# qwerfdsaplking/SATrans

Measured on AMD Instinct MI355X. Metric: training samples/sec (AliCCP-shaped, emb=32, 3L/4H, meta_mode=QK), higher is better.
Workload: dtype f32; 1 GPU; BASELINE configs[1]: AliCCP-shaped SATrans training step, 19 fields, 6,571,961 table rows (841 MB fp32), uniform ids, dropout on, dense-Adam+L2 semantics over all rows; batch_per_gpu=8192, global_batch=8192, embedding_dim=32, layers=3, heads=4, fields=19, parallelism=dp1

## Files before the change

### satrans_amd/csrc/embed_adam.hip

```cpp
#include <algorithm>
#include <cstdlib>
#include <cstring>

#include <rocprim/rocprim.hpp>

#include "common.h"

namespace satrans {

constexpr int kChunk = 16;
constexpr int kStreamBlock = 256;
constexpr int kStreamBlocks = 2048;

struct AdamK {
    float neg_step, w1, beta2, w2, eps, l2x2, l2;
    double rbc2;
    float rbc2f;
    int fast;
};

__host__ inline AdamK make_adamk(const satrans_adam_hparams& h) {
    AdamK k;
    k.neg_step = -h.lr_over_bc1;
    k.rbc2 = 1.0 / (double)h.bc2_sqrt;
// ... 268 lines not shown
__device__ __forceinline__ void touched_apply_body(int64_t bid, double* s_red, float4* __restrict__ P, float4* __restrict__ M,
                                                   float4* __restrict__ V, const int32_t* __restrict__ sorted_rows,
                                                   int64_t n, const float4* __restrict__ rowsum,
                                                   const int32_t* __restrict__ head_of, const AdamK& k,
                                                   double* __restrict__ reg_partials, float4* __restrict__ G,
                                                   int32_t* __restrict__ last, int t) {
    const int64_t j = (bid * 256 + threadIdx.x) / LPR;
    const int q = threadIdx.x % LPR;
    double reg = 0.0;
    if (j < n && head_of[j] == 1) {
        const int64_t at = (int64_t)sorted_rows[j] * LPR + q;
        if (G) {
            G[at] = rowsum[j * LPR + q];
        } else {
            float4 p = P[at], m = M[at], v = V[at];
            reg += adam4(p, m, v, rowsum[j * LPR + q], k);
            P[at] = p; M[at] = m; V[at] = v;
            if (last && q == 0) last[sorted_rows[j]] = t;
        }
    }
    const double total = block_sum(reg, s_red);
    if (threadIdx.x == 0) reg_partials[bid] = total;
}

template <int LPR>
__device__ __forceinline__ void touched_finish_body(int64_t bid, double* s_red, float4* __restrict__ P, float4* __restrict__ M,
                                                    float4* __restrict__ V, int64_t chunks,
                                                    const float4* __restrict__ done_sum,
                                                    const int32_t* __restrict__ done_row, const AdamK& k,
                                                    double* __restrict__ reg_partials, float4* __restrict__ G,
                                                    int32_t* __restrict__ last, int t) {
    const int64_t c = (bid * 256 + threadIdx.x) / LPR;
    const int q = threadIdx.x % LPR;
    double reg = 0.0;
    if (c < chunks) {
        const int32_t row = done_row[c];
        if (row >= 0) {
            const int64_t at = (int64_t)row * LPR + q;
            if (G) {
                G[at] = done_sum[c * LPR + q];
            } else {
                float4 p = P[at], m = M[at], v = V[at];
                reg += adam4(p, m, v, done_sum[c * LPR + q], k);
                P[at] = p; M[at] = m; V[at] = v;
                if (last && q == 0) last[row] = t;
            }
        }
    }
    const double total = block_sum(reg, s_red);
    if (threadIdx.x == 0) reg_partials[bid] = total;
}

template <int LPR>
__device__ __forceinline__ void touched_spans_body(int64_t bid, double* s_red, float4* __restrict__ P, float4* __restrict__ M,
                                                   float4* __restrict__ V, int64_t chunks,
                                                   const float4* __restrict__ partial,
                                                   const int32_t* __restrict__ info,
                                                   const int32_t* __restrict__ trail_row, const AdamK& k,
                                                   double* __restrict__ reg_partials, float4* __restrict__ G,
                                                   int32_t* __restrict__ last, int t) {
    const int64_t group = (bid * 256 + threadIdx.x) / LPR;
    const int q = threadIdx.x % LPR;
    double reg = 0.0;
    if (group < chunks && (info[group] & 1)) {
        float4 acc = partial[(group * 2 + 1) * LPR + q];
        for (int64_t c = group + 1; c < chunks; ++c) {
            const int f = info[c];
            if (!(f & 2)) break;
            const float4 g = partial[(c * 2 + 0) * LPR + q];
            acc.x += g.x; acc.y += g.y; acc.z += g.z; acc.w += g.w;
            if (f & 4) break;
        }
        const int64_t at = (int64_t)trail_row[group] * LPR + q;
        if (G) {
            G[at] = acc;
        } else {
            float4 p = P[at], m = M[at], v = V[at];
            reg += adam4(p, m, v, acc, k);
            P[at] = p; M[at] = m; V[at] = v;
            if (last && q == 0) last[trail_row[group]] = t;
        }
    }
    const double total = block_sum(reg, s_red);
    if (threadIdx.x == 0) reg_partials[bid] = total;
}

template <int LPR>
__global__ __launch_bounds__(256) void touched_step_kernel(int64_t sblocks, int64_t cblocks, float4* __restrict__ P,
                                                          float4* __restrict__ M, float4* __restrict__ V, AdamK k,
                                                          float4* __restrict__ G, int32_t* __restrict__ last, int t,
                                                          const int32_t* __restrict__ sorted_rows, int64_t n,
                                                          const float4* __restrict__ rowsum, const int32_t* __restrict__ head_of,
                                                          double* __restrict__ reg_apply, int64_t chunks,
                                                          const float4* __restrict__ done_sum, const int32_t* __restrict__ done_row,
                                                          double* __restrict__ reg_finish, int64_t supers,
                                                          const float4* __restrict__ partial2, const int32_t* __restrict__ info2,
                                                          const int32_t* __restrict__ trail_row2, double* __restrict__ reg_spans) {
    __builtin_amdgcn_s_setprio(3);
    __shared__ double s_red[256];
    const int64_t b = blockIdx.x;
    if (b < sblocks)
        touched_spans_body<LPR>(b, s_red, P, M, V, supers, partial2, info2, trail_row2, k, reg_spans, G, last, t);
    else if (b < sblocks + cblocks)
        touched_finish_body<LPR>(b - sblocks, s_red, P, M, V, chunks, done_sum, done_row, k, reg_finish, G, last, t);
    else
        touched_apply_body<LPR>(b - sblocks - cblocks, s_red, P, M, V, sorted_rows, n, rowsum, head_of, k, reg_apply, G, last, t);
}

template <int LPR>
__global__ __launch_bounds__(256) void adam_rows_kernel(float4* __restrict__ P, float4* __restrict__ M,
                                                       float4* __restrict__ V, int64_t row0, int64_t rows,
                                                       const float4* __restrict__ G, int32_t* __restrict__ last, int t,
                                                       AdamK k, double* __restrict__ reg_partials) {
    __shared__ double s_red[256];
    const int64_t i = (int64_t)blockIdx.x * 256 + threadIdx.x;
    double reg = 0.0;
    if (i < rows * LPR) {
        const int64_t at = row0 * LPR + i;
        float4 p = P[at], m = M[at], v = V[at];
        reg = adam4(p, m, v, G[i], k);
        P[at] = p; M[at] = m; V[at] = v;
        if (last && i % LPR == 0) last[row0 + i / LPR] = t;
    }
    const double total = block_sum(reg, s_red);
    if (threadIdx.x == 0) reg_partials[blockIdx.x] = total;
}

template <int LPR>
__global__ void pack_rows_kernel(const int32_t* __restrict__ src, int64_t n, const float4* __restrict__ gemb,
                                 float4* __restrict__ out) {
    const int64_t i = (int64_t)blockIdx.x * blockDim.x + threadIdx.x;
    if (i >= n * LPR) return;
    out[i] = gemb[(int64_t)src[i / LPR] * LPR + i % LPR];
}


struct LazyK {
    float w1, beta2, w2, eps, l2x2, l2;
    int fast;
};
__host__ inline LazyK make_lazyk(const satrans_adam_hparams& h) {
    LazyK k;
    k.fast = h.arith == SATRANS_ADAM_FAST ? 1 : 0;
    k.w1 = (float)(1.0 - (double)h.beta1);
    k.beta2 = h.beta2;
    k.w2 = (float)(1.0 - (double)h.beta2);
    k.eps = h.eps;
    k.l2 = h.l2;
    k.l2x2 = 2.0f * h.l2;
    return k;
}

using f32x2 = __attribute__((ext_vector_type(2))) float;

__device__ __forceinline__ f32x2 pk_fma(f32x2 a, f32x2 b, f32x2 c) { return __builtin_elementwise_fma(a, b, c); }
__device__ __forceinline__ f32x2 pk_mul(f32x2 a, f32x2 b) {
#pragma clang fp contract(off)
    return a * b;
}
__device__ __forceinline__ f32x2 pk_add(f32x2 a, f32x2 b) {
#pragma clang fp contract(off)
    return a + b;
}
__device__ __forceinline__ f32x2 pk_sub(f32x2 a, f32x2 b) {
#pragma clang fp contract(off)
    return a - b;
}
__device__ __forceinline__ f32x2 pk_set(float x) { return f32x2{x, x}; }

constexpr float kPkVLo = 0x1p-100f, kPkVHi = 0x1p64f;
constexpr float kPkALo = 0x1p-80f, kPkAHi = 0x1p40f;
constexpr float kPkEpsLo = 0x1p-30f;

__device__ __forceinline__ f32x2 pk_sqrt_rn(f32x2 x) {
    const f32x2 r = {__builtin_amdgcn_rsqf(x.x), __builtin_amdgcn_rsqf(x.y)};
    f32x2 s = pk_mul(x, r);
    f32x2 h = pk_mul(r, pk_set(0.5f));
    const f32x2 e = pk_fma(-h, s, pk_set(0.5f));
    h = pk_fma(h, e, h);
    s = pk_fma(s, e, s);
    const f32x2 d = pk_fma(-s, s, x);
    return pk_fma(d, h, s);
}

__device__ __forceinline__ f32x2 pk_div_rn(f32x2 a, f32x2 b) {
    f32x2 r = {__builtin_amdgcn_rcpf(b.x), __builtin_amdgcn_rcpf(b.y)};
    const f32x2 e = pk_fma(-b, r, pk_set(1.0f));
    r = pk_fma(e, r, r);
    f32x2 q = pk_mul(a, r);
    f32x2 d = pk_fma(-b, q, a);
    q = pk_fma(d, r, q);
    d = pk_fma(-b, q, a);
    return pk_fma(d, r, q);
}

__device__ __forceinline__ f32x2 pk_sqrt_ext(f32x2 v) {
    const bool sx = v.x < kPkVLo, sy = v.y < kPkVLo;
    const f32x2 up = {sx ? 0x1p64f : 1.0f, sy ? 0x1p64f : 1.0f};
    const f32x2 dn = {sx ? 0x1p-32f : 1.0f, sy ? 0x1p-32f : 1.0f};
    return pk_mul(pk_sqrt_rn(pk_mul(v, up)), dn);
}

__device__ __forceinline__ f32x2 pk_div_ext(f32x2 a, f32x2 den, bool& redo_x, bool& redo_y) {
    const bool sx = fabsf(a.x) < kPkALo, sy = fabsf(a.y) < kPkALo;
    const f32x2 up = {sx ? 0x1p69f : 1.0f, sy ? 0x1p69f : 1.0f};
    const f32x2 dn = {sx ? 0x1p-69f : 1.0f, sy ? 0x1p-69f : 1.0f};
    const f32x2 qs = pk_div_rn(pk_mul(a, up), den);
    f32x2 q = pk_mul(qs, dn);
    redo_x = sx && a.x != 0.f && !(fabsf(qs.x) >= 0x1p-57f);
    redo_y = sy && a.y != 0.f && !(fabsf(qs.y) >= 0x1p-57f);
    q.x = a.x == 0.f ? a.x : q.x;
    q.y = a.y == 0.f ? a.y : q.y;
    return q;
}

__device__ __forceinline__ float denom_of(float root, double rbc2, float eps) {
    return __fadd_rn((float)__dmul_rn((double)root, rbc2), eps);
}

__device__ __forceinline__ void adam_step4(f32x2 (&p)[2], f32x2 (&m)[2], f32x2 (&v)[2], f32x2 (&sq)[2], float neg_step,
                                           double rbc2, const LazyK& k) {
    f32x2 a[2];
#pragma unroll
    for (int u = 0; u < 2; ++u) {
        sq[u] = pk_fma(p[u], p[u], sq[u]);
        const f32x2 g = pk_add(pk_set(0.f), pk_mul(pk_set(k.l2x2), p[u]));
        m[u] = pk_fma(pk_set(k.w1), pk_sub(g, m[u]), m[u]);
        v[u] = pk_fma(pk_mul(pk_set(k.w2), g), g, pk_mul(v[u], pk_set(k.beta2)));
        a[u] = pk_mul(pk_set(neg_step), m[u]);
    }
    const float vmin = fminf(__builtin_fminf(__builtin_fminf(v[0].x, v[0].y), v[1].x), v[1].y);
    const float vmax = fmaxf(__builtin_fmaxf(__builtin_fmaxf(v[0].x, v[0].y), v[1].x), v[1].y);
    const float amin = fminf(__builtin_fminf(__builtin_fminf(fabsf(a[0].x), fabsf(a[0].y)), fabsf(a[1].x)), fabsf(a[1].y));
    const float amax = fmaxf(__builtin_fmaxf(__builtin_fmaxf(fabsf(a[0].x), fabsf(a[0].y)), fabsf(a[1].x)), fabsf(a[1].y));
    const bool packed = vmin >= kPkVLo && vmax <= kPkVHi && amin >= kPkALo && amax <= kPkAHi && k.eps >= kPkEpsLo;
    if (__all(packed)) {
#pragma unroll
        for (int u = 0; u < 2; ++u) {
            const f32x2 root = pk_sqrt_rn(v[u]);
            const f32x2 den = {denom_of(root.x, rbc2, k.eps), denom_of(root.y, rbc2, k.eps)};
            p[u] = pk_add(p[u], pk_div_rn(a[u], den));
        }
        return;
    }
    const bool v_sane = v[0].x >= 0.f && v[0].y >= 0.f && v[1].x >= 0.f && v[1].y >= 0.f;
    if (__all(k.eps > 0.f && v_sane && a[0].x == 0.f && a[0].y == 0.f && a[1].x == 0.f && a[1].y == 0.f)) {
        p[0] = pk_add(p[0], a[0]);
        p[1] = pk_add(p[1], a[1]);
        return;
    }
    const bool lane_small = amax < 0x1p-60f;
    auto lane_ok = [&](float a_) { return lane_small || a_ == 0.f || fabsf(a_) >= kPkALo; };
    const bool by_lane = v_sane && vmin >= kPkVLo && vmax <= kPkVHi && amax <= kPkAHi && k.eps >= kPkEpsLo && lane_ok(a[0].x) &&
                         lane_ok(a[0].y) && lane_ok(a[1].x) && lane_ok(a[1].y);
    if (__all(by_lane)) {
        const f32x2 up = pk_set(lane_small ? 0x1p69f : 1.0f), dn = pk_set(lane_small ? 0x1p-69f : 1.0f);
        f32x2 q[2], den[2];
#pragma unroll
        for (int u = 0; u < 2; ++u) {
            const f32x2 root = pk_sqrt_rn(v[u]);
            den[u] = f32x2{denom_of(root.x, rbc2, k.eps), denom_of(root.y, rbc2, k.eps)};
            q[u] = pk_mul(pk_div_rn(pk_mul(a[u], up), den[u]), dn);
        }
        if (lane_small && fmaxf(fmaxf(den[0].x, den[0].y), fmaxf(den[1].x, den[1].y)) > 0x1p-23f) {
#pragma unroll
            for (int u = 0; u < 2; ++u) q[u] = f32x2{__fdiv_rn(a[u].x, den[u].x), __fdiv_rn(a[u].y, den[u].y)};
        }
#pragma unroll
        for (int u = 0; u < 2; ++u) {
            q[u].x = a[u].x == 0.f ? a[u].x : q[u].x;
            q[u].y = a[u].y == 0.f ? a[u].y : q[u].y;
            p[u] = pk_add(p[u], q[u]);
        }
        return;
    }
    auto ext_ok = [&](float a_, float v_) { return (a_ == 0.f && v_ >= 0.f) || (fabsf(a_) <= kPkAHi && v_ > 0.f && v_ <= kPkVHi); };
    const bool extended = ext_ok(a[0].x, v[0].x) && ext_ok(a[0].y, v[0].y) && ext_ok(a[1].x, v[1].x) && ext_ok(a[1].y, v[1].y) &&
                          k.eps >= kPkEpsLo;
    if (__all(extended)) {
#pragma unroll
        for (int u = 0; u < 2; ++u) {
            const f32x2 root = pk_sqrt_ext(v[u]);
            const f32x2 den = {denom_of(root.x, rbc2, k.eps), denom_of(root.y, rbc2, k.eps)};
            bool redo_x, redo_y;
            f32x2 q = pk_div_ext(a[u], den, redo_x, redo_y);
            if (redo_x) q.x = __fdiv_rn(a[u].x, den.x);
            if (redo_y) q.y = __fdiv_rn(a[u].y, den.y);
            p[u] = pk_add(p[u], q);
        }
        return;
    }
#pragma unroll
    for (int u = 0; u < 2; ++u) {
        p[u].x = __fadd_rn(p[u].x, __fdiv_rn(a[u].x, denom_of(sqrtf(v[u].x), rbc2, k.eps)));
        p[u].y = __fadd_rn(p[u].y, __fdiv_rn(a[u].y, denom_of(sqrtf(v[u].y), rbc2, k.eps)));
    }
}

__device__ __forceinline__ void adam_step4_fast(f32x2 (&p)[2], f32x2 (&m)[2], f32x2 (&v)[2], f32x2 (&sq)[2], float neg_step,
                                                float rbc2f, const LazyK& k) {
#pragma unroll
    for (int u = 0; u < 2; ++u) {
        sq[u] = pk_fma(p[u], p[u], sq[u]);
        const f32x2 g = pk_add(pk_set(0.f), pk_mul(pk_set(k.l2x2), p[u]));
        m[u] = pk_fma(pk_set(k.w1), pk_sub(g, m[u]), m[u]);
        v[u] = pk_fma(pk_mul(pk_set(k.w2), g), g, pk_mul(v[u], pk_set(k.beta2)));
        const f32x2 a = pk_mul(pk_set(neg_step), m[u]);
        const f32x2 root = {__builtin_amdgcn_sqrtf(v[u].x), __builtin_amdgcn_sqrtf(v[u].y)};
        const f32x2 den = pk_fma(root, pk_set(rbc2f), pk_set(k.eps));
        const f32x2 r = {__builtin_amdgcn_rcpf(den.x), __builtin_amdgcn_rcpf(den.y)};
        p[u] = pk_fma(a, r, p[u]);
    }
}

__device__ __forceinline__ double replay_element4(float4& P4, float4& M4, float4& V4, int from, int to,
                                                  const double2* __restrict__ table, const LazyK& k) {
    f32x2 p[2] = {{P4.x, P4.y}, {P4.z, P4.w}}, m[2] = {{M4.x, M4.y}, {M4.z, M4.w}}, v[2] = {{V4.x, V4.y}, {V4.z, V4.w}};
    f32x2 sq[2] = {{0.f, 0.f}, {0.f, 0.f}};
    if (k.fast) {
        for (int s = from + 1; s <= to; ++s) {
            const double2 hp = table[s];
            adam_step4_fast(p, m, v, sq, -(float)hp.x, (float)hp.y, k);
        }
    } else {
        for (int s = from + 1; s <= to; ++s) {
            const double2 hp = table[s];
            adam_step4(p, m, v, sq, -(float)hp.x, hp.y, k);
        }
    }
    P4 = make_float4(p[0].x, p[0].y, p[1].x, p[1].y);
    M4 = make_float4(m[0].x, m[0].y, m[1].x, m[1].y);
    V4 = make_float4(v[0].x, v[0].y, v[1].x, v[1].y);
    return (double)k.l2 * (((double)sq[0].x + (double)sq[0].y) + ((double)sq[1].x + (double)sq[1].y));
}

template <int D>
__global__ __launch_bounds__(256) void lazy_replay_kernel(float4* __restrict__ P, float4* __restrict__ M, float4* __restrict__ V,
                                                         int32_t* __restrict__ last, const int32_t* __restrict__ sorted_rows,
                                                         int64_t n, int target, const double2* __restrict__ table, LazyK k,
                                                         double* __restrict__ reg_partials, int64_t slots) {
    constexpr int LR = D / 4;
    __shared__ double s_red[256];
    const int64_t j = ((int64_t)blockIdx.x * 256 + threadIdx.x) / LR;
    const int c = threadIdx.x % LR;
    double reg = 0.0;
    if (j < n) {
        const int32_t row = sorted_rows[j];
        const bool head = j == 0 || sorted_rows[j - 1] != row;
        if (head) {
            const int from = last[row];
            if (from < target) {
                const int64_t at = (int64_t)row * LR + c;
                float4 p = P[at], m = M[at], v = V[at];
                reg = replay_element4(p, m, v, from, target, table, k);
                P[at] = p; M[at] = m; V[at] = v;
            }
        }
    }
    __syncthreads();
    if (j < n && c == 0) {
        const int32_t row = sorted_rows[j];
        if ((j == 0 || sorted_rows[j - 1] != row) && last[row] < target) last[row] = target;
    }
    const double total = block_sum(reg, s_red);
    if (threadIdx.x == 0) {
        reg_partials[blockIdx.x] = total;
        for (int64_t t = (int64_t)blockIdx.x + gridDim.x; t < slots; t += gridDim.x) reg_partials[t] = 0.0;
    }
}

template <int D>
__global__ __launch_bounds__(256) void lazy_flush_kernel(float4* __restrict__ P, float4* __restrict__ M, float4* __restrict__ V,
                                                        int32_t* __restrict__ last, int64_t total_rows, int target,
                                                        const double2* __restrict__ table, LazyK k,
                                                        double* __restrict__ reg_partials) {
    constexpr int LR = D / 4;
    __shared__ double s_red[256];
    double reg = 0.0;
    const int64_t groups_per_pass = (int64_t)gridDim.x * 256 / LR;
    const int c = threadIdx.x % LR;
    for (int64_t row = ((int64_t)blockIdx.x * 256 + threadIdx.x) / LR; row < total_rows; row += groups_per_pass) {
        const int from = last[row];
        if (from < target) {
            const int64_t at = row * LR + c;
            float4 p = P[at], m = M[at], v = V[at];
            reg += replay_element4(p, m, v, from, target, table, k);
            P[at] = p; M[at] = m; V[at] = v;
        }
    }
    __syncthreads();
    for (int64_t row = ((int64_t)blockIdx.x * 256 + threadIdx.x) / LR; row < total_rows; row += groups_per_pass)
        if (c == 0 && last[row] < target) last[row] = target;
    const double total = block_sum(reg, s_red);
    if (threadIdx.x == 0) reg_partials[blockIdx.x] = total;
}

__global__ void packed_math_check_kernel(int mode, uint64_t first, uint64_t count, unsigned long long* __restrict__ bad) {
    unsigned long long mine = 0;
    for (uint64_t i = (uint64_t)blockIdx.x * blockDim.x + threadIdx.x; i < count; i += (uint64_t)gridDim.x * blockDim.x) {
        if (mode == 2) {
            const float x = __uint_as_float((uint32_t)(first + i));
            if (!(x > 0.f && x < kPkVLo)) continue;
            const f32x2 r = pk_sqrt_ext(f32x2{x, x});
            const float want = (float)sqrt((double)x);
            mine += (__float_as_uint(r.x) != __float_as_uint(want)) + (__float_as_uint(r.y) != __float_as_uint(want));
        } else if (mode == 3) {
            uint64_t z = (first + i) * 0x9E3779B97F4A7C15ull + 0xD1B54A32D192ED03ull;
            z = (z ^ (z >> 30)) * 0xBF58476D1CE4E5B9ull;
            z = (z ^ (z >> 27)) * 0x94D049BB133111EBull;
            z ^= z >> 31;
            uint64_t w = (z + 0x9E3779B97F4A7C15ull) * 0xBF58476D1CE4E5B9ull;
            w ^= w >> 29;
            const uint32_t ea = (uint32_t)((w >> 8) % 48u);
            const uint32_t eb = 127 - 30 + (uint32_t)((w >> 20) % 68u);
            float a = __uint_as_float(((uint32_t)(w & 1u) << 31) | (ea << 23) | (uint32_t)(z & 0x7FFFFFu));
            if ((w >> 40) % 64u == 0) a = __uint_as_float((uint32_t)(w & 1u) << 31);
            const float b = __uint_as_float((eb << 23) | (uint32_t)((z >> 23) & 0x7FFFFFu));
            bool rx, ry;
            f32x2 q = pk_div_ext(f32x2{a, -a}, f32x2{b, b}, rx, ry);
            if (rx) q.x = __fdiv_rn(a, b);
            if (ry) q.y = __fdiv_rn(-a, b);
            const float want = (float)((double)a / (double)b);
            mine += __float_as_uint(__fdiv_rn(a, b)) != __float_as_uint(want);
            mine += (__float_as_uint(q.x) != __float_as_uint(want)) + (__float_as_uint(q.y) != __float_as_uint(-want));
        } else if (mode == 0) {
            const float x = __uint_as_float((uint32_t)(first + i));
            if (!(x >= kPkVLo && x <= kPkVHi)) continue;
            const f32x2 r = pk_sqrt_rn(f32x2{x, x});
            const float want = (float)sqrt((double)x);
            mine += __float_as_uint(sqrtf(x)) != __float_as_uint(want);
            mine += (__float_as_uint(r.x) != __float_as_uint(want)) + (__float_as_uint(r.y) != __float_as_uint(want));
        } else {
            uint64_t z = (first + i) * 0x9E3779B97F4A7C15ull + 0xD1B54A32D192ED03ull;
            z = (z ^ (z >> 30)) * 0xBF58476D1CE4E5B9ull;
            z = (z ^ (z >> 27)) * 0x94D049BB133111EBull;
            z ^= z >> 31;
            uint64_t w = (z + 0x9E3779B97F4A7C15ull) * 0xBF58476D1CE4E5B9ull;
            w ^= w >> 29;
            const uint32_t ea = 127 - 80 + (uint32_t)((w >> 8) % 120u);
            const uint32_t eb = 127 - 30 + (uint32_t)((w >> 20) % 68u);
            const float a = __uint_as_float(((uint32_t)(w & 1u) << 31) | (ea << 23) | (uint32_t)(z & 0x7FFFFFu));
            const float b = __uint_as_float((eb << 23) | (uint32_t)((z >> 23) & 0x7FFFFFu));
            const f32x2 q = pk_div_rn(f32x2{a, -a}, f32x2{b, b});
            const float want = (float)((double)a / (double)b);
            mine += __float_as_uint(__fdiv_rn(a, b)) != __float_as_uint(want);
            mine += (__float_as_uint(q.x) != __float_as_uint(want)) + (__float_as_uint(q.y) != __float_as_uint(-want));
        }
    }
    if (mine) atomicAdd(bad, mine);
}

__global__ void mark_last_kernel(const int32_t* __restrict__ sorted_rows, int64_t n, int32_t* __restrict__ last, int t) {
    const int64_t j = (int64_t)blockIdx.x * blockDim.x + threadIdx.x;
    if (j >= n) return;
    const int32_t row = sorted_rows[j];
    if (j == 0 || sorted_rows[j - 1] != row) last[row] = t;
}

template <int LPR>
__global__ void grad_dense_kernel(const int32_t* __restrict__ sorted_rows, const int32_t* __restrict__ src, int64_t n,
                                  const float4* __restrict__ gemb, float4* __restrict__ g_arena) {
    const int64_t j0 = ((int64_t)blockIdx.x * blockDim.x + threadIdx.x) / LPR;
    const int q = threadIdx.x % LPR;
    if (j0 >= n) return;
    const int32_t row = sorted_rows[j0];
    if (j0 > 0 && sorted_rows[j0 - 1] == row) return;
    float4 acc = make_float4(0.f, 0.f, 0.f, 0.f);
    for (int64_t j = j0; j < n && sorted_rows[j] == row; ++j) {
        const float4 g = gemb[(int64_t)src[j] * LPR + q];
        acc.x += g.x; acc.y += g.y; acc.z += g.z; acc.w += g.w;
    }
    float4 out = g_arena[(int64_t)row * LPR + q];
    out.x += acc.x; out.y += acc.y; out.z += acc.z; out.w += acc.w;
    g_arena[(int64_t)row * LPR + q] = out;
}

__global__ void add_l2_grad_kernel(const float* __restrict__ p, float* __restrict__ g, int64_t n, float l2x2) {
    const int64_t i = (int64_t)blockIdx.x * blockDim.x + threadIdx.x;
    if (i < n) g[i] += l2x2 * p[i];
}

__global__ void adam_flat_kernel(float* __restrict__ p, const float* __restrict__ g, float* __restrict__ m,
                                 float* __restrict__ v, int64_t n, AdamK k) {
    const int64_t i = (int64_t)blockIdx.x * blockDim.x + threadIdx.x;
    if (i >= n) return;
    float pp = p[i], mm = m[i], vv = v[i];
    adam1(pp, mm, vv, __fadd_rn(g[i], __fmul_rn(k.l2x2, pp)), k);
    p[i] = pp; m[i] = mm; v[i] = vv;
}

__device__ __forceinline__ double strided_sum_1024(const double* __restrict__ vals, int64_t count) {
    constexpr int kDeep = 16;
    double acc = 0.0;
    int64_t i = threadIdx.x;
    for (; i + (kDeep - 1) * 1024 < count; i += kDeep * 1024) {
        double t[kDeep];
#pragma unroll
        for (int u = 0; u < kDeep; ++u) t[u] = vals[i + u * 1024];
#pragma unroll
        for (int u = 0; u < kDeep; ++u) acc += t[u];
    }
    if (i < count) {
        double t[kDeep];
#pragma unroll
        for (int u = 0; u < kDeep; ++u) t[u] = vals[min(i + (int64_t)u * 1024, count - 1)];
#pragma unroll
        for (int u = 0; u < kDeep; ++u)
            if (i + (int64_t)u * 1024 < count) acc += t[u];
    }
    return acc;
}

__global__ __launch_bounds__(1024) void adam_flat_sum_kernel(float* __restrict__ p, const float* __restrict__ g,
                                                           float* __restrict__ m, float* __restrict__ v, int64_t n, AdamK k,
                                                           const double* __restrict__ vals, int64_t count,
                                                           double* __restrict__ out) {
    __builtin_amdgcn_s_setprio(3);
    __shared__ double s_red[1024];
    if (blockIdx.x + 1 < gridDim.x) {
        const int64_t i = (int64_t)blockIdx.x * blockDim.x + threadIdx.x;
        if (i >= n) return;
        float pp = p[i], mm = m[i], vv = v[i];
        adam1(pp, mm, vv, __fadd_rn(g[i], __fmul_rn(k.l2x2, pp)), k);
        p[i] = pp; m[i] = mm; v[i] = vv;
        return;
    }
    const double total = block_sum(strided_sum_1024(vals, count), s_red);
    if (threadIdx.x == 0) out[0] += total;
}

__global__ __launch_bounds__(1024) void sum_f64_kernel(const double* __restrict__ vals, int64_t count,
                                                      double* __restrict__ out, int accumulate) {
    __shared__ double s_red[1024];
    const double acc = strided_sum_1024(vals, count);
    const double total = block_sum(acc, s_red);
    if (threadIdx.x == 0) out[0] = accumulate ? out[0] + total : total;
}

static int bits_for(int64_t n) {
    int bits = 1;
    while (((int64_t)1 << bits) < n) ++bits;
    return bits;
}

struct SortLayout {
    size_t keys_in, pos_in, temp, temp_bytes, total;
};
static SortLayout sort_layout(int64_t n, int64_t total_rows) {
    SortLayout L{};
    auto align = [](size_t x) { return (x + 255) & ~(size_t)255; };
    size_t temp = 0;
    (void)rocprim::radix_sort_pairs(nullptr, temp, (const uint32_t*)nullptr, (uint32_t*)nullptr, (const int32_t*)nullptr,
                              (int32_t*)nullptr, (unsigned)n, 0u, (unsigned)bits_for(total_rows), (hipStream_t)0);
    L.keys_in = 0;
    L.pos_in = align(sizeof(uint32_t) * (size_t)n);
    L.temp = align(L.pos_in + sizeof(int32_t) * (size_t)n);
    L.temp_bytes = temp;
    L.total = align(L.temp + temp);
    return L;
}

static int64_t touched_blocks(int64_t n, int D) {
    const int lpr = D / 4;
    return ceil_div(n * lpr, 256);
}
static int64_t chunk_blocks(int64_t n, int D) {
    const int lpr = D / 4;
    return ceil_div(ceil_div(n, kChunk) * lpr, 256);
}

}

using namespace satrans;

#define DISPATCH_LPR(D, CALL)                                                        \
    switch ((D) / 4) {                                                               \
        case 4: { constexpr int LPR = 4; CALL; } break;                              \
        case 8: { constexpr int LPR = 8; CALL; } break;                              \
        case 16: { constexpr int LPR = 16; CALL; } break;                            \
        case 32: { constexpr int LPR = 32; CALL; } break;                            \
        default:                                                                     \
            ::satrans::set_error("embedding_dim %d not in {16,32,64,128}", (D));     \
            return SATRANS_E_UNSUPPORTED;                                            \
    }

extern "C" int64_t satrans_embed_sort_workspace_bytes(int64_t n, int64_t total_rows) {
    if (n <= 0 || total_rows <= 0) return 0;
    return (int64_t)sort_layout(n, total_rows).total;
}

extern "C" int satrans_embed_sort(const int32_t* rows, int64_t n, int64_t total_rows, int32_t* sorted_rows, int32_t* src,
                                  uint32_t* touched, void* workspace, int64_t workspace_bytes, const int32_t* positions,
                                  void* stream_) {
    hipStream_t stream = (hipStream_t)stream_;
    SATRANS_REQUIRE(rows && sorted_rows && src && workspace, SATRANS_E_BADARG, "embed_sort: null pointer");
    SATRANS_REQUIRE(n > 0 && total_rows > 0 && n < ((int64_t)1 << 31) && total_rows < ((int64_t)1 << 31), SATRANS_E_BADARG,
                    "embed_sort: sizes n=%lld rows=%lld", (long long)n, (long long)total_rows);
    const SortLayout L = sort_layout(n, total_rows);
    SATRANS_REQUIRE((int64_t)L.total <= workspace_bytes, SATRANS_E_WORKSPACE, "embed_sort: workspace %lld < %lld bytes",
                    (long long)workspace_bytes, (long long)L.total);
    char* ws = (char*)workspace;
    uint32_t* keys_in = (uint32_t*)(ws + L.keys_in);
    int32_t* pos_in = (int32_t*)(ws + L.pos_in);
    hipError_t e = hipSuccess;
    if (touched) e = hipMemsetAsync(touched, 0, sizeof(uint32_t) * (size_t)ceil_div(total_rows, 32), stream);
    SATRANS_REQUIRE(e == hipSuccess, SATRANS_E_LAUNCH, "embed_sort: memset: %s", hipGetErrorString(e));
    const uint32_t* keys = keys_in;
    const int32_t* pos = pos_in;
    if (positions) {
        keys = (const uint32_t*)rows;
        pos = positions;
    } else {
        iota_kernel<<<(unsigned)ceil_div(n, 256), 256, 0, stream>>>(rows, n, keys_in, pos_in);
        SATRANS_CHECK_LAUNCH("iota_kernel");
    }
    size_t temp_bytes = L.temp_bytes;
    e = rocprim::radix_sort_pairs(ws + L.temp, temp_bytes, keys, (uint32_t*)sorted_rows, pos, src, (unsigned)n, 0u,
                                  (unsigned)bits_for(total_rows), stream);
    SATRANS_REQUIRE(e == hipSuccess, SATRANS_E_LAUNCH, "embed_sort: radix sort: %s", hipGetErrorString(e));
    if (touched) {
        mark_heads_kernel<<<(unsigned)ceil_div(n, 256), 256, 0, stream>>>(sorted_rows, n, touched);
        SATRANS_CHECK_LAUNCH("mark_heads_kernel");
    }
    return SATRANS_OK;
}

constexpr int kMergeRunsMax = 64;
struct MergeRuns {
    int32_t start[kMergeRunsMax + 1];
};
__global__ __launch_bounds__(256) void merge_runs_kernel(const int32_t* __restrict__ ids, int n, int W, MergeRuns R,
                                                         int32_t* __restrict__ sorted_rows, int32_t* __restrict__ src) {
    const int i = blockIdx.x * 256 + threadIdx.x;
    if (i >= n) return;
    const int32_t x = ids[i];
    int r = 0;
    while (r + 1 < W && i >= R.start[r + 1]) ++r;
    int pos = i - R.start[r];
    for (int q0 = 0; q0 < W; q0 += 8) {
        int lo[8], hi[8];
#pragma unroll
        for (int k = 0; k < 8; ++k) {
            const int q = q0 + k;
            const bool on = q < W && q != r;
            lo[k] = on ? R.start[q] : 0;
            hi[k] = on ? R.start[q + 1] : 0;
        }
        bool more = true;
        while (more) {
            more = false;
#pragma unroll
            for (int k = 0; k < 8; ++k) {
                if (lo[k] < hi[k]) {
                    const int mid = (lo[k] + hi[k]) >> 1;
                    const int32_t v = ids[mid];
                    const bool right = (q0 + k < r) ? (v <= x) : (v < x);
                    if (right) lo[k] = mid + 1; else hi[k] = mid;
                    more = true;
                }
            }
        }
#pragma unroll
        for (int k = 0; k < 8; ++k) {
            const int q = q0 + k;
            if (q < W && q != r) pos += lo[k] - R.start[q];
        }
    }
    sorted_rows[pos] = x;
    src[pos] = i;
}

extern "C" int satrans_embed_merge_runs(const int32_t* ids, int64_t n, const int64_t* h_run_start, int W, int32_t* sorted_rows,
                                        int32_t* src, void* stream_) {
    hipStream_t stream = (hipStream_t)stream_;
    SATRANS_REQUIRE(ids && h_run_start && sorted_rows && src, SATRANS_E_BADARG, "embed_merge_runs: null pointer");
    SATRANS_REQUIRE(W >= 1 && W <= kMergeRunsMax, SATRANS_E_UNSUPPORTED, "embed_merge_runs: %d runs (1..%d)", W, kMergeRunsMax);
    SATRANS_REQUIRE(n >= 0 && n < ((int64_t)1 << 31) && h_run_start[0] == 0 && h_run_start[W] == n, SATRANS_E_BADARG,
                    "embed_merge_runs: run boundaries do not cover [0, %lld)", (long long)n);
    MergeRuns R;
    for (int q = 0; q <= kMergeRunsMax; ++q) R.start[q] = (int32_t)h_run_start[std::min(q, W)];
    for (int q = 0; q < W; ++q)
        SATRANS_REQUIRE(R.start[q] <= R.start[q + 1], SATRANS_E_BADARG, "embed_merge_runs: run %d has a negative length", q);
    if (n == 0) return SATRANS_OK;
    merge_runs_kernel<<<(unsigned)ceil_div(n, 256), 256, 0, stream>>>(ids, (int)n, W, R, sorted_rows, src);
    SATRANS_CHECK_LAUNCH("merge_runs_kernel");
    return SATRANS_OK;
}

__global__ __launch_bounds__(256) void inverse_positions_kernel(const int32_t* __restrict__ src, int n, int32_t* __restrict__ inv) {
    const int i = blockIdx.x * 256 + threadIdx.x;
    if (i < n) inv[src[i]] = i;
// ... 405 lines not shown
```

Measured before the change: 8.910 million samples/s.

## Stage recent Adam step coefficients in LDS and replay wave-uniformly

Lazy Adam replay kernels now preload the last 128 per-step coefficients (converted to float) into shared memory. When a wavefront's minimum pending step falls in that window, all lanes loop over the same step range and read the coefficients from LDS, with inactive lanes masked by a per-lane check. Otherwise they fall back to the global table. The flush loop is restructured so whole waves stay converged. The goal is to remove per-step global loads and divergent loop trip counts. The cost is extra masked iterations for lanes with shorter histories, plus a block barrier at kernel start.

```diff
diff --git a/satrans_amd/csrc/embed_adam.hip b/satrans_amd/csrc/embed_adam.hip
--- a/satrans_amd/csrc/embed_adam.hip
+++ b/satrans_amd/csrc/embed_adam.hip
@@ -594,7 +594,7 @@
 #pragma unroll
     for (int u = 0; u < 2; ++u) {
         sq[u] = pk_fma(p[u], p[u], sq[u]);
-        const f32x2 g = pk_add(pk_set(0.f), pk_mul(pk_set(k.l2x2), p[u]));
+        const f32x2 g = pk_mul(pk_set(k.l2x2), p[u]);
         m[u] = pk_fma(pk_set(k.w1), pk_sub(g, m[u]), m[u]);
         v[u] = pk_fma(pk_mul(pk_set(k.w2), g), g, pk_mul(v[u], pk_set(k.beta2)));
         const f32x2 a = pk_mul(pk_set(neg_step), m[u]);
@@ -605,14 +605,39 @@
     }
 }
 
+constexpr int kStagedSteps = 128;
+
+__device__ __forceinline__ void stage_steps(float2* s_steps, int target, const double2* __restrict__ table) {
+    const int s = target - (int)threadIdx.x;
+    if (threadIdx.x < kStagedSteps && s >= 1) {
+        const double2 hp = table[s];
+        s_steps[threadIdx.x] = make_float2(-(float)hp.x, (float)hp.y);
+    }
+    __syncthreads();
+}
+
+__device__ __forceinline__ int wave_min(int x) {
+#pragma unroll
+    for (int off = 32; off > 0; off >>= 1) x = min(x, __shfl_xor(x, off));
+    return __builtin_amdgcn_readfirstlane(x);
+}
+
 __device__ __forceinline__ double replay_element4(float4& P4, float4& M4, float4& V4, int from, int to,
-                                                  const double2* __restrict__ table, const LazyK& k) {
+                                                  const double2* __restrict__ table, const float2* s_steps, const LazyK& k) {
     f32x2 p[2] = {{P4.x, P4.y}, {P4.z, P4.w}}, m[2] = {{M4.x, M4.y}, {M4.z, M4.w}}, v[2] = {{V4.x, V4.y}, {V4.z, V4.w}};
     f32x2 sq[2] = {{0.f, 0.f}, {0.f, 0.f}};
     if (k.fast) {
-        for (int s = from + 1; s <= to; ++s) {
-            const double2 hp = table[s];
-            adam_step4_fast(p, m, v, sq, -(float)hp.x, (float)hp.y, k);
+        const int first = wave_min(from) + 1;
+        if (first >= 1 && to - first < kStagedSteps) {
+            for (int s = first; s <= to; ++s) {
+                const float2 c = s_steps[to - s];
+                if (s > from) adam_step4_fast(p, m, v, sq, c.x, c.y, k);
+            }
+        } else {
+            for (int s = from + 1; s <= to; ++s) {
+                const double2 hp = table[s];
+                adam_step4_fast(p, m, v, sq, -(float)hp.x, (float)hp.y, k);
+            }
         }
     } else {
         for (int s = from + 1; s <= to; ++s) {
@@ -633,22 +658,25 @@
                                                          double* __restrict__ reg_partials, int64_t slots) {
     constexpr int LR = D / 4;
     __shared__ double s_red[256];
+    __shared__ float2 s_steps[kStagedSteps];
+    if (k.fast) stage_steps(s_steps, target, table);
     const int64_t j = ((int64_t)blockIdx.x * 256 + threadIdx.x) / LR;
     const int c = threadIdx.x % LR;
-    double reg = 0.0;
+    int from = target;
+    int64_t at = 0;
     if (j < n) {
         const int32_t row = sorted_rows[j];
         const bool head = j == 0 || sorted_rows[j - 1] != row;
         if (head) {
-            const int from = last[row];
-            if (from < target) {
-                const int64_t at = (int64_t)row * LR + c;
-                float4 p = P[at], m = M[at], v = V[at];
-                reg = replay_element4(p, m, v, from, target, table, k);
-                P[at] = p; M[at] = m; V[at] = v;
-            }
-        }
-    }
+            from = min(last[row], target);
+            at = (int64_t)row * LR + c;
+        }
+    }
+    const bool work = from < target;
+    float4 p = make_float4(0.f, 0.f, 0.f, 0.f), m = p, v = p;
+    if (work) { p = P[at]; m = M[at]; v = V[at]; }
+    const double reg = replay_element4(p, m, v, from, target, table, s_steps, k);
+    if (work) { P[at] = p; M[at] = m; V[at] = v; }
     __syncthreads();
     if (j < n && c == 0) {
         const int32_t row = sorted_rows[j];
@@ -668,17 +696,21 @@
                                                         double* __restrict__ reg_partials) {
     constexpr int LR = D / 4;
     __shared__ double s_red[256];
+    __shared__ float2 s_steps[kStagedSteps];
+    if (k.fast) stage_steps(s_steps, target, table);
     double reg = 0.0;
     const int64_t groups_per_pass = (int64_t)gridDim.x * 256 / LR;
     const int c = threadIdx.x % LR;
-    for (int64_t row = ((int64_t)blockIdx.x * 256 + threadIdx.x) / LR; row < total_rows; row += groups_per_pass) {
-        const int from = last[row];
-        if (from < target) {
-            const int64_t at = row * LR + c;
-            float4 p = P[at], m = M[at], v = V[at];
-            reg += replay_element4(p, m, v, from, target, table, k);
-            P[at] = p; M[at] = m; V[at] = v;
-        }
+    const int first_lane = (int)(threadIdx.x & ~63u);
+    for (int64_t row0 = ((int64_t)blockIdx.x * 256 + first_lane) / LR; row0 < total_rows; row0 += groups_per_pass) {
+        const int64_t row = row0 + (threadIdx.x - first_lane) / LR;
+        const int from = row < total_rows ? min(last[row], target) : target;
+        const bool work = from < target;
+        const int64_t at = row * LR + c;
+        float4 p = make_float4(0.f, 0.f, 0.f, 0.f), m = p, v = p;
+        if (work) { p = P[at]; m = M[at]; v = V[at]; }
+        reg += replay_element4(p, m, v, from, target, table, s_steps, k);
+        if (work) { P[at] = p; M[at] = m; V[at] = v; }
     }
     __syncthreads();
     for (int64_t row = ((int64_t)blockIdx.x * 256 + threadIdx.x) / LR; row < total_rows; row += groups_per_pass)
```

New measurement: 9.080 million samples/s (median of 6 runs). 1.02x the previous value.
